# jfjell/Octree-Raymarcher

Hardware: AMD Instinct MI355X
Metric: Mrays/s (primary+shadow) at 1920x1080, depth-12 SVO (higher is better)
Workload: dtype f32; 1 GPU; c3_1080p_depth12_4x1x4_shadow; depth_per_chunk=12, chunksize=128, nodes=99473656, bricks=34206642, hbm_pool_bytes=11087035656, kernel=auto, launches_in_flight=2, frames_per_launch=16, frames_in_flight=32, gather=False, partition=single, ranks_seen=1, launcher=single process

## Files before the change

include/svo.h:

```cpp
#ifndef SVO_H
#define SVO_H

#include <stdint.h>
#include <stddef.h>

#ifdef __cplusplus
extern "C" {
#endif

#define SVO_ABI_VERSION 4

typedef enum svo_status {
    SVO_OK                 =  0,
    SVO_OK_LITERAL_ONLY    =  1,
    SVO_ERR_INVALID_ARG    = -1,
    SVO_ERR_NO_DEVICE      = -2,
    SVO_ERR_OUT_OF_MEMORY  = -3,
    SVO_ERR_MALFORMED_TREE = -4,
    SVO_ERR_NOT_UPLOADED   = -5,
    SVO_ERR_UNSUPPORTED    = -6,
    SVO_ERR_HIP            = -7
} svo_status;

enum { SVO_EMPTY = 0, SVO_LEAF = 1, SVO_BRANCH = 2, SVO_TWIG = 3 };
// ... 51 lines not shown
    int32_t  max_tree_steps;
    int32_t  max_twig_steps;
    int32_t  shadow;
    float    light_dir[3];
    int32_t  kernel;
    int32_t  tiles_per_wave;
    uint32_t *counters_dev;
    int32_t  normal_mode;
    int32_t  launches_in_flight;
    uint32_t       *tile_cost_dev;
    const uint32_t *tile_order_dev;
    int32_t  semantics;
    uint32_t see_through;
} svo_trace_params;
enum { SVO_NORMAL_CUBE = 0, SVO_NORMAL_FACE = 1 };
enum { SVO_SHADOW_NO_CLEARANCE = 2 };
enum { SVO_SEMANTICS_CPU = 0, SVO_SEMANTICS_GLSL = 1 };

enum {
    SVO_HIT_FLAG      = 1u << 0,
    SVO_SHADOW_TRACED = 1u << 1,
    SVO_SHADOWED      = 1u << 2,
    SVO_FACE_NORMAL   = 1u << 3,
    SVO_SEE_THROUGH   = 1u << 4,
    SVO_LOCAL_SHADOWS  = 1u << 5,
    SVO_SHADOWED_POINT = 1u << 6,
    SVO_SHADOWED_SPOT  = 1u << 7,
    SVO_ERR_FLAG      = 1u << 15
};
#define SVO_CELL_NONE 0xFFu

// ... 207 lines not shown
    float    alpha;
    uint32_t style;
    uint32_t _pad[3];
} svo_box;

int svo_cursor_place(const float origin[3], const float dir[3], const svo_hit *record_dev,
                     float size, svo_box *box_dev, void *stream);

int svo_shade_boxes(const svo_camera *cam, const svo_box *boxes_dev, int nboxes, float near_plane, float far_plane,
                    int x0, int y0, int w, int h, float *rgba_dev, void *stream);

int svo_trace_last_ray_count(svo_world *, void *stream, uint64_t *rays);

int svo_world_prepare_light(svo_world *, const float light_dir[3], void *stream);
int svo_world_prepared_light(svo_world *, void *stream, float shadow_dir[3], uint64_t *clear_nodes);

int   svo_device_count(void);
void *svo_device_alloc(size_t bytes);
void  svo_device_free(void *p_dev);
void  svo_device_cache_trim(void);
int   svo_memcpy_h2d(void *dst_dev, const void *src, size_t bytes);
int   svo_memcpy_d2h(void *dst, const void *src_dev, size_t bytes);
int   svo_stream_synchronize(void *stream);

const char *svo_last_error(void);
int         svo_abi_version(void);

#ifdef __cplusplus
}
#endif
// ... 2 lines not shown
```

octree-raymarcher_amd/__init__.py:

```python
from __future__ import annotations

import ctypes as C
import math
import os
from typing import Optional, Sequence

import numpy as np

from . import partition

_HERE = os.path.dirname(os.path.abspath(__file__))
LIB_PATH = os.environ.get("SVO_AMD_LIB") or os.path.join(_HERE, "libsvo_amd.so")

if not os.path.exists(LIB_PATH):
    raise ImportError(
        f"{LIB_PATH} is missing: build it with `make -C {_HERE}` (or __graft_entry__.build()). "
        "There is no CPU fallback for the SVO march.")

lib = C.CDLL(LIB_PATH)

SVO_OK = 0
OK_LITERAL_ONLY = 1
ERR_NAMES = {0: "SVO_OK", -1: "SVO_ERR_INVALID_ARG", -2: "SVO_ERR_NO_DEVICE", -3: "SVO_ERR_OUT_OF_MEMORY",
             -4: "SVO_ERR_MALFORMED_TREE", -5: "SVO_ERR_NOT_UPLOADED", -6: "SVO_ERR_UNSUPPORTED", -7: "SVO_ERR_HIP"}
EMPTY, LEAF, BRANCH, TWIG = 0, 1, 2, 3
KERNEL_AUTO, KERNEL_LITERAL, KERNEL_STACK = 0, 1, 2
EDIT_BUILD, EDIT_DESTROY, EDIT_REPLACE = 0, 1, 2
HIT_FLAG, SHADOW_TRACED, SHADOWED, FACE_NORMAL, SEE_THROUGH, ERR_FLAG = 1, 2, 4, 8, 16, 1 << 15
LOCAL_SHADOWS, SHADOWED_POINT, SHADOWED_SPOT = 1 << 5, 1 << 6, 1 << 7
NORMAL_CUBE, NORMAL_FACE = 0, 1
SHADOW_NO_CLEARANCE = 2
SEMANTICS_CPU, SEMANTICS_GLSL = 0, 1
CELL_NONE = 0xFF
SKY_LINEAR, SKY_NEAREST = 0, 1
BOX_SOLID, BOX_CURSOR, BOX_HIDDEN = 0, 1, 1 << 8
MAX_BOXES = 64
BOX_DTYPE = np.dtype([("bmin", "<f4", (3,)), ("size", "<f4"), ("color", "<f4", (3,)), ("alpha", "<f4"), ("style", "<u4"), ("_pad", "<u4", (3,))])
assert BOX_DTYPE.itemsize == 48

HIT_DTYPE = np.dtype([("t", "<f4"), ("normal", "<f4", (3,)), ("material", "<u2"), ("flags", "<u2"),
                      ("chunk", "<u4"), ("node", "<u4"), ("cell", "<u4")])
assert HIT_DTYPE.itemsize == 32
LOCATE_INSIDE, LOCATE_SOLID = 1, 2
VOXEL_DTYPE = np.dtype([("bmin", "<f4", (3,)), ("size", "<f4"), ("material", "<u2"), ("flags", "<u2"),
                        ("chunk", "<u4"), ("node", "<u4"), ("cell", "<u4")])
assert VOXEL_DTYPE.itemsize == 32
# ... 99 lines not shown
                ("total_trees", C.c_uint64), ("total_twigs", C.c_uint64),
                ("tree_pool_bytes", C.c_uint64), ("twig_pool_bytes", C.c_uint64), ("mask_pool_bytes", C.c_uint64),
                ("max_chunk_depth", C.c_int32), ("exact_geometry", C.c_int32),
                ("wide_pool_bytes", C.c_uint64), ("wide_nodes", C.c_uint64)]


MAX_FRAMES = 16

ABI_SYMBOLS = [
    "svo_world_generate", "svo_world_create", "svo_world_info_get", "svo_world_chunk", "svo_world_destroy",
    "svo_world_index_float", "svo_world_index", "svo_world_locate", "svo_hit_voxels", "svo_hit_uv", "svo_shade_textured", "svo_world_upload", "svo_world_update",
    "svo_chunk_from_grid", "svo_world_chunk_from_grid", "svo_world_chunk_to_grid",
    "svo_chunk_write", "svo_chunk_read", "svo_chunk_free", "svo_world_shift", "svo_world_edit_box", "svo_world_edit_cube", "svo_world_edit_ball", "svo_world_edit_ball_all", "svo_world_compact", "svo_world_coarsen", "svo_shade", "svo_shade_packed", "svo_shade_translucent", "svo_shade_sky", "svo_frame_rgba8", "svo_cursor_place", "svo_shade_boxes", "svo_shade_defaults", "svo_gbuffer_pack", "svo_gbuffer_unpack",
    "svo_tile_order", "svo_trace", "svo_trace_rows", "svo_trace_frames", "svo_trace_rows_frames", "svo_trace_rays", "svo_trace_segments", "svo_trace_translucent", "svo_trace_local_shadows", "svo_trace_last_ray_count",
    "svo_shadowmap_fit", "svo_shadowmap_render", "svo_shadowmap_apply", "svo_hit_ao", "svo_shade_ao",
    "svo_trace_reflections", "svo_shade_reflections", "svo_world_prepare_light", "svo_world_prepared_light",
    "svo_device_count", "svo_device_alloc", "svo_device_free", "svo_device_cache_trim", "svo_memcpy_h2d", "svo_memcpy_d2h",
    "svo_stream_synchronize", "svo_last_error", "svo_abi_version",
]

_P = C.c_void_p
lib.svo_last_error.restype = C.c_char_p
lib.svo_abi_version.restype = C.c_int
lib.svo_world_edit_box.argtypes = [_P, C.c_int, C.c_int, C.POINTER(C.c_float), C.POINTER(C.c_float), C.c_uint16]
lib.svo_world_edit_cube.argtypes = [_P, C.c_int, C.POINTER(C.c_float), C.c_float, C.c_uint16, C.POINTER(C.c_int), C.POINTER(C.c_int)]
lib.svo_world_edit_ball.argtypes = [_P, C.c_int, C.c_int, C.POINTER(C.c_float), C.c_float, C.c_uint16]
lib.svo_world_edit_ball_all.argtypes = [_P, C.c_int, C.POINTER(C.c_float), C.c_float, C.c_uint16, C.POINTER(C.c_int), C.c_int, C.POINTER(C.c_int)]
lib.svo_world_compact.argtypes = [_P, C.c_int]
lib.svo_world_compact.restype = C.c_int
lib.svo_world_coarsen.argtypes = [_P, C.c_int]
lib.svo_world_coarsen.restype = C.c_int
# ... 38 lines not shown
lib.svo_world_locate.argtypes = [_P, _P, C.c_int64, C.POINTER(TraceParams), _P, _P]
lib.svo_hit_voxels.argtypes = [_P, _P, C.c_int64, _P, _P]
lib.svo_hit_uv.argtypes = [C.POINTER(Camera), C.c_float, C.c_int, C.c_int, C.c_int, C.c_int, _P, _P, _P, _P]
lib.svo_shade_textured.argtypes = [C.POINTER(Camera), C.POINTER(ShadeParams), C.POINTER(Atlas), C.c_int, C.c_int, C.c_int, C.c_int, _P, _P, _P, _P]
lib.svo_hit_ao.argtypes = [_P, C.POINTER(Camera), C.POINTER(TraceParams), C.c_float, C.c_int, C.c_int, C.c_int, C.c_int, _P, _P, _P, _P]
lib.svo_shade_ao.argtypes = [_P, C.c_float, C.c_int64, _P, _P]
lib.svo_trace_reflections.argtypes = [_P, C.POINTER(Camera), C.POINTER(TraceParams), C.c_uint32, C.c_int, C.c_int, C.c_int, C.c_int, _P, _P, _P, _P]
lib.svo_shade_reflections.argtypes = [C.POINTER(Camera), C.POINTER(ShadeParams), C.POINTER(Mirror), C.c_int, C.c_int, C.c_int, C.c_int, _P, _P, _P, _P, _P]
lib.svo_shade_sky.argtypes = [C.POINTER(Camera), C.POINTER(Sky), C.c_int, C.c_int, C.c_int, C.c_int, _P, _P, _P, _P]
lib.svo_frame_rgba8.argtypes = [_P, C.c_int64, _P, _P]
lib.svo_cursor_place.argtypes = [C.POINTER(C.c_float), C.POINTER(C.c_float), _P, C.c_float, _P, _P]
lib.svo_shade_boxes.argtypes = [C.POINTER(Camera), _P, C.c_int, C.c_float, C.c_float, C.c_int, C.c_int, C.c_int, C.c_int, _P, _P]
lib.svo_trace_last_ray_count.argtypes = [_P, _P, C.POINTER(C.c_uint64)]
lib.svo_world_prepare_light.argtypes = [_P, C.POINTER(C.c_float), _P]
lib.svo_world_prepared_light.argtypes = [_P, _P, C.POINTER(C.c_float), C.POINTER(C.c_uint64)]
lib.svo_device_count.restype = C.c_int
lib.svo_device_alloc.argtypes = [C.c_size_t]
lib.svo_device_alloc.restype = _P
lib.svo_device_free.argtypes = [_P]
lib.svo_device_free.restype = None
lib.svo_device_cache_trim.argtypes = []
lib.svo_device_cache_trim.restype = None
lib.svo_memcpy_h2d.argtypes = [_P, _P, C.c_size_t]
lib.svo_memcpy_d2h.argtypes = [_P, _P, C.c_size_t]
lib.svo_stream_synchronize.argtypes = [_P]


def _check(rc: int, where: str) -> int:
    if rc < 0:
        raise SvoError(rc, where)
# ... 62 lines not shown
def default_camera(world_w: int, world_d: int, chunksize: int, width: int, height: int) -> Camera:
    cx = world_w * chunksize * 0.5
    return make_camera((cx, 150.0, -40.0), (0.0, -0.5, 0.866), (0.0, 1.0, 0.0), 60.0, width, height)


def c5_scene() -> dict:
    return {
        "generate": dict(pyramid_resolution=4096, water=False, coarse_depth=10, refine_box=((62.0, -1e9, -1e9), (66.0, 1e9, 1e9))),
        "camera": lambda w, h: make_camera((64.3, 12.7, 96.5), (0.0, -0.8, 0.6), (0.0, 1.0, 0.0), 60.0, w, h),
    }


def trace_params(shadow: bool = False, kernel: int = KERNEL_AUTO, light_dir=(1.0, -1.0, 0.0), eps: float = 0.0,
                 caps=(0, 0, 0), counters_dev: Optional[int] = None, tiles_per_wave: int = 0, normal_mode: int = 0,
                 tile_cost_dev: Optional[int] = None, tile_order_dev: Optional[int] = None, launches_in_flight: int = 0,
                 semantics: int = 0, see_through: int = 0, light_clearance: bool = True) -> TraceParams:
    p = TraceParams()
    p.semantics = semantics
    p.see_through = see_through
    p.normal_mode = normal_mode
    p.eps = eps
    p.max_chunk_steps, p.max_tree_steps, p.max_twig_steps = caps
    p.shadow = (1 if light_clearance else 1 | SHADOW_NO_CLEARANCE) if shadow else 0
    p.light_dir[:] = [float(x) for x in light_dir]
    p.kernel = kernel
    p.counters_dev = counters_dev
    p.tiles_per_wave = tiles_per_wave
    p.tile_cost_dev = tile_cost_dev
    p.tile_order_dev = tile_order_dev
    p.launches_in_flight = launches_in_flight
    return p


def chunk_write(path: str, chunk: dict, treestoragesize: int = 0, twigstoragesize: int = 0):
    tree = np.ascontiguousarray(chunk["tree"], dtype=np.uint32)
    twig = np.ascontiguousarray(chunk["twig"], dtype=np.uint16)
    d = ChunkDesc()
    d.position[:] = [float(x) for x in chunk["position"]]
# ... 337 lines not shown

    def shadowmap_render(self, smap: ShadowMap, params: TraceParams, stream: int = 0):
        _check(lib.svo_shadowmap_render(self._h, C.byref(smap) if smap is not None else None, C.byref(params) if params is not None else None,
                                        stream), "svo_shadowmap_render")

    def tile_order(self, cost_ptr: int, order_ptr: int, ntiles: int, stream: int = 0):
        _check(lib.svo_tile_order(self._h, cost_ptr, order_ptr, ntiles, stream), "svo_tile_order")

    def prepare_light(self, light_dir=(1.0, -1.0, 0.0), stream: int = 0):
        _check(lib.svo_world_prepare_light(self._h, (C.c_float * 3)(*[float(v) for v in light_dir]), stream), "svo_world_prepare_light")

    def prepared_light(self, stream: int = 0):
        sdir, n = (C.c_float * 3)(), C.c_uint64()
        _check(lib.svo_world_prepared_light(self._h, stream, sdir, C.byref(n)), "svo_world_prepared_light")
        return tuple(sdir), n.value

    def last_ray_count(self, stream: int = 0) -> int:
        n = C.c_uint64()
        _check(lib.svo_trace_last_ray_count(self._h, stream, C.byref(n)), "svo_trace_last_ray_count")
        return n.value

    def draw(self, cam: Camera, rect=None, shadow: bool = False, kernel: int = KERNEL_AUTO, counters: bool = False,
             light_dir=(1.0, -1.0, 0.0), normal_mode: int = 0, semantics: int = 0, see_through: int = 0, local_shadows=None, shadowmap=None):
        x0, y0, w, h = rect if rect is not None else (0, 0, cam.width, cam.height)
        out = DeviceBuffer(max(w * h, 1) * 32)
        cnt = DeviceBuffer(max(w * h, 1) * 16) if counters else None
        prm = trace_params(shadow=shadow, kernel=kernel, light_dir=light_dir, counters_dev=cnt.ptr if cnt else None, normal_mode=normal_mode,
                           semantics=semantics, see_through=see_through)
        if shadowmap is not None:
            prm.shadow = 0
# ... 120 lines not shown
```

octree-raymarcher_amd/csrc/device.hip:

```cpp
#include <hip/hip_runtime.h>

#include <algorithm>
#include <cmath>
#include <cstdlib>
#include <chrono>
#include <cstring>
#include <mutex>
#include <new>
#include <string>
#include <vector>

#include "kernel_literal.hip.h"
#include "kernel_stack.hip.h"
#include "see_through.hip.h"
#include "local_shadows.hip.h"
#include "reflect.hip.h"
#include "shadowmap.hip.h"
#include "locate.hip.h"
#include "ao.hip.h"
#include "hit_voxels.hip.h"
#include "hip_own.h"
#include "wide_tree.hip.h"
#include "light_clearance.hip.h"

// ... 12 lines not shown
#pragma unroll
    for (int k = 0; k < 4; ++k) {
        const uint32_t a = w[k] & 0xFFFFu, b = w[k] >> 16;
        bits |= (a ? 1u : 0u) << (2 * k);
        bits |= (b ? 1u : 0u) << (2 * k + 1);
        if (a) { lo = a < lo ? a : lo; hi = a > hi ? a : hi; }
        if (b) { lo = b < lo ? b : lo; hi = b > hi ? b : hi; }
    }
#pragma unroll
    for (int d = 1; d < 8; d <<= 1) {
        const uint32_t lo2 = __shfl_xor(lo, d, 64), hi2 = __shfl_xor(hi, d, 64);
        lo = lo2 < lo ? lo2 : lo; hi = hi2 > hi ? hi2 : hi;
    }
    if (!live) return;
    reinterpret_cast<uint8_t *>(mask + first)[i] = (uint8_t)bits;
    if ((i & 7u) == 0u) bmat[first + (i >> 3)] = (uint16_t)(hi == 0u ? 0u : (lo == hi ? lo : 0xFFFFu));
}

__global__ __launch_bounds__(256) void k_tile_keys(const uint32_t *cost, uint32_t *keys, uint32_t *idx, int n)
{
    const int i = blockIdx.x * 256 + threadIdx.x;
    if (i >= n) return;
    const uint32_t a = cost[2 * i], b = cost[2 * i + 1];
    keys[i] = a + b < a ? 0xFFFFFFFFu : a + b;
    idx[i] = (uint32_t)i;
}

constexpr size_t POOL_CACHE_SLOTS = 8, POOL_CACHE_MIN = 1u << 20;
struct PoolBuf { void *p; size_t bytes; int device; };
static std::mutex g_pool_mutex;
static std::vector<PoolBuf> g_pool_cache;
// ... 49 lines not shown
    w.hbm->view_wide = Pooled<uint32_t>(); w.hbm->view_mask = Pooled<uint64_t>(); w.hbm->view_material = 0;
}

static void drop_parents(svo_world &w)
{
    Hbm &d = *w.hbm;
    if (d.parent.p || d.parent_level.p || d.chunk_trees.p) (void)hipDeviceSynchronize();
    d.parent = Pooled<uint32_t>(); d.parent_level = Pooled<uint8_t>(); d.chunk_trees = DevBuf<uint32_t>();
    d.parents_ok = false;
}

static void drop_clearance(svo_world &w)
{
    Hbm &d = *w.hbm;
    if (d.clear_place.p) { (void)hipDeviceSynchronize(); d.clear_place = Pooled<uint4>(); }
    d.clear_state = Hbm::CLEAR_DROPPED; d.clear_usable = false;
}

int release_device(svo_world &w, bool keep_builder)
{
    if (w.hbm) {
        (void)hipSetDevice(w.device);
        drop_view(w);
        drop_parents(w);
        if (!keep_builder) free_builder_context(w);
        (void)hipDeviceSynchronize();
        delete w.hbm;
        w.hbm = nullptr;
    }
    w.device = -1;
    w.table.clear(); w.tree_slot.clear(); w.twig_slot.clear(); w.wtable.clear(); w.wide_slot.clear();
// ... 696 lines not shown
    float m = 1.0f;
    for (int a = 0; a < 3; ++a)
        for (int k = 0; k < 2; ++k) m = std::max(m, std::fabs((float)(w.chunkcoordmin[a] + k * dims[a]) * (float)w.chunksize));
    return std::nextafter(m, INFINITY) - m;
}
static bool eps_is_pow2(float eps)
{
    uint32_t b;
    std::memcpy(&b, &eps, sizeof b);
    return (b & 0x807FFFFFu) == 0u && b >= 0x00800000u && b < 0x7F800000u;
}

static int prepare_light(svo_world &w, const float sdir[3], hipStream_t s)
{
    Hbm &d = *w.hbm;
    d.clear_usable = false;
    if (!w.wide_ok || w.wide_pool_len == 0) return SVO_OK;
    HIP_TRY(hipSetDevice(w.device));
    bool premises = true;
    for (int a = 0; a < 3; ++a) premises &= std::isfinite(sdir[a]) && (sdir[a] == 0.0f || std::fabs((double)sdir[a]) >= CLEAR_S_MIN);
    std::memcpy(d.clear_sdir, sdir, sizeof d.clear_sdir);
    d.clear_state = Hbm::CLEAR_READY;
    if (!premises || !w.exact_geometry) return SVO_OK;
    d.clear_state = Hbm::CLEAR_DROPPED;
    const uint64_t nodes = w.wide_pool_len;
    if (d.clear_place.bytes < nodes * sizeof(uint4)) {
        if (d.clear_place.p) HIP_TRY(hipDeviceSynchronize());
        if (d.clear_place.alloc(nodes, w.device) != hipSuccess) { set_error("svo_world_prepare_light: hipMalloc failed"); return SVO_ERR_OUT_OF_MEMORY; }
    }
    if (const int rc = d.clear_count.reserve(1, false, nullptr)) return rc;
    for (Event &e : d.work_done) if (e.e) if (const int rc = e.wait(s)) return rc;
    if (d.clear_built.e) if (const int rc = d.clear_built.wait(s)) return rc;
    const double u = (double)clear_spacing(w);
    ClearArgs K;
    K.wchunks = d.wchunks.p; K.wide = d.wide.p; K.place = d.clear_place.p; K.pool_nodes = nodes;
    K.n_chunks = (int32_t)w.chunks.size(); K.chunksize = (double)w.chunksize;
    for (int a = 0; a < 3; ++a) K.s[a] = (double)sdir[a];
    K.d1 = 4.0 * u;
    K.d2 = (8.0 / CLEAR_S_MIN + 6.0 + 4.0 * (double)(w.width + w.height + w.depth + 2)) * u;
    K.clear_nodes = d.clear_count.p;
    HIP_TRY(hipMemsetAsync(d.clear_place.p, 0xFF, nodes * sizeof(uint4), s));
    HIP_TRY(hipMemsetAsync(d.clear_count.p, 0, sizeof(unsigned long long), s));
    int rc = launch_per_element("svo_world_prepare_light", K.n_chunks, s, k_clear_seed, K);
    const int nw_max = w.max_levels ? (w.max_levels + 1) / 2 : 1;
    for (int r = 0; rc == SVO_OK && r + 1 < nw_max; ++r) rc = launch_per_element("svo_world_prepare_light", (int64_t)nodes * 64, s, k_clear_boxes, K, (uint32_t)r);
    if (rc == SVO_OK) rc = launch_per_element("svo_world_prepare_light", (int64_t)nodes * 64, s, k_clear_sweep, K);
    if (rc != SVO_OK) return rc;
    if ((rc = d.clear_built.record(s)) != SVO_OK) return rc;
    d.clear_state = Hbm::CLEAR_READY;
    d.clear_usable = true;
    d.clear_eps = 2.0f * (float)u;
    return SVO_OK;
}

static int use_light_clearance(svo_world *w, const svo_trace_params *prm, TraceArgs &A, uint32_t see, hipStream_t s)
{
    A.light_clear = 0;
    if (!A.shadow || !A.from_camera || A.tmax || see || A.glsl || A.tile_cost || (prm && (prm->shadow & SVO_SHADOW_NO_CLEARANCE))) return SVO_OK;
    Hbm &d = *w->hbm;
    if (d.clear_state == Hbm::CLEAR_FRESH && (double)w->wide_pool_len * 64.0 * (double)w->chunks.size() <= CLEAR_AUTO_WORK)
        if (const int rc = prepare_light(*w, A.sdir, s)) return rc;
    if (d.clear_state != Hbm::CLEAR_READY || !d.clear_usable) return SVO_OK;
    if (std::memcmp(d.clear_sdir, A.sdir, sizeof d.clear_sdir) != 0 || !eps_is_pow2(A.eps) || A.eps < d.clear_eps) return SVO_OK;
    if (const int rc = d.clear_built.wait(s)) return rc;
    A.light_clear = 1;
    return SVO_OK;
}

static int launch(svo_world *w, const svo_trace_params *prm, TraceArgs &A, hipStream_t s)
{
    const int kernel = pick_kernel(w, prm, A);
    if (kernel < 0) return kernel;
    HIP_TRY(hipSetDevice(w->device));
    const uint32_t see = prm ? prm->see_through : 0u;
    if (see && kernel == SVO_KERNEL_STACK) {
        const int rc = use_view(w, see, A, s);
        if (rc != SVO_OK) return rc;
    }
    if (kernel == SVO_KERNEL_STACK) if (const int rc = use_light_clearance(w, prm, A, see, s)) return rc;
    Hbm &d = *w->hbm;
// ... 438 lines not shown
    const Hbm &d = *w->hbm;
    shadow_dir[0] = shadow_dir[1] = shadow_dir[2] = 0.0f;
    *clear_nodes = 0;
    if (d.clear_state != Hbm::CLEAR_READY) return SVO_OK;
    std::memcpy(shadow_dir, d.clear_sdir, sizeof d.clear_sdir);
    if (!d.clear_usable) return SVO_OK;
    HIP_TRY(hipSetDevice(w->device));
    HIP_TRY(hipStreamSynchronize((hipStream_t)stream));
    if (d.clear_built.e) HIP_TRY(hipEventSynchronize(d.clear_built.e));
    unsigned long long v = 0;
    HIP_TRY(hipMemcpy(&v, d.clear_count.p, sizeof v, hipMemcpyDeviceToHost));
    *clear_nodes = v;
    return SVO_OK;
}

}
```

octree-raymarcher_amd/csrc/hip_own.h:

```cpp
#pragma once
#include <hip/hip_runtime.h>

#include <algorithm>
#include <cstring>
#include <string>
#include <utility>
#include <vector>

#include "world.h"

namespace svo {

inline int hip_status(hipError_t e)
{
    return e == hipErrorOutOfMemory ? SVO_ERR_OUT_OF_MEMORY : (e == hipErrorNoDevice || e == hipErrorInvalidDevice) ? SVO_ERR_NO_DEVICE : SVO_ERR_HIP;
}
#define HIP_TRY(expr)                                                                              \
    do { if (hipError_t e_ = (expr); e_ != hipSuccess) { svo::set_error(std::string(#expr) + ": " + hipGetErrorString(e_)); return svo::hip_status(e_); } } while (0)

inline unsigned blocks_for(uint64_t n, unsigned per) { return (unsigned)((n + per - 1) / per); }

inline int launch_status(const char *who)
{
    const hipError_t e = hipGetLastError();
// ... 139 lines not shown
    Event work_done[WORK_SLOTS];
    OrderedScratch<unsigned char> sort;
    OrderedScratch<float> cont;
    OrderedScratch<float> mirror;
    OrderedScratch<float> local;
    OrderedScratch<float> shadowmap;
    Pooled<uint32_t> view_wide; Pooled<uint64_t> view_mask;
    uint32_t view_material = 0;
    Event view_built;
    Pooled<uint32_t> parent; Pooled<uint8_t> parent_level; DevBuf<uint32_t> chunk_trees;
    bool parents_ok = false;
    Event parents_built;
    enum { CLEAR_FRESH = 0, CLEAR_READY = 1, CLEAR_DROPPED = 2 };
    int clear_state = CLEAR_FRESH;
    bool clear_usable = false;
    float clear_sdir[3] = { 0.0f, 0.0f, 0.0f }; float clear_eps = 0.0f;
    Pooled<uint4> clear_place; DevBuf<unsigned long long> clear_count;
    Event clear_built;
    int stack_blocks[24] = {};
};

}
```

octree-raymarcher_amd/csrc/kernel_stack.hip.h:

```cpp
#pragma once
#include "march.hip.h"
#include "step_asm.hip.h"

namespace svo {

constexpr int CW_ESCAPE_PENDING = (int)0x80000000;
enum : int { M_DONE = 0, M_WORLD = 1, M_HIT = 2, M_TREE = 3, M_TWIG = 4 };

constexpr int VOTE_WORLD = 8;
constexpr int VOTE_HIT = 16;
constexpr int VOTE_BUSY = 24;
constexpr int CREEP_SERIOUS = 6;
constexpr int CREEP_LANES = 8;
#define SVO_LIKELY(x) __builtin_expect(!!(x), 1)
#define SVO_UNLIKELY(x) __builtin_expect(!!(x), 0)
constexpr int STEP_EXTRA = 4;
constexpr int STEP_LANES = 8;
constexpr int DRAIN_STEPS = 8;
#ifndef SVO_SURE_MISS_WHEN
#define SVO_SURE_MISS_WHEN __builtin_amdgcn_readfirstlane(more ? 0 : 1)
#endif

__device__ __forceinline__ float recip_pow2(float x) { return __uint_as_float(0x7F000000u - __float_as_uint(x)); }

// ... 582 lines not shown
                node = wb[child ? 0u : 1u + ci] + (child ? ci : gi);
            }
            const uint32_t hitc = (uint32_t)cnt;
            V3 vlo;
            float vsize;
            uint32_t material;
            if (hitc == SVO_CELL_NONE) {
                const int low = (1 << (levels - plev)) - 1;
                vlo = mk(Blo.x + (float)(pux & ~low) * res, Blo.y + (float)(puy & ~low) * res, Blo.z + (float)(puz & ~low) * res);
                vsize = res * (float)(low + 1);
                material = word & 0xFFFFu;
            } else {
                vlo = mk(Blo.x + (float)(hitc & 3u) * res, Blo.y + (float)((hitc >> 2) & 3u) * res, Blo.z + (float)(hitc >> 4) * res);
                vsize = res;
                const unsigned long long brick = (unsigned long long)twig_off + (word & WIDE_PAYLOAD);
                material = A.bmat[brick];
                if (material == 0xFFFFu) material = A.twig[brick * TWIG_WORDS + hitc];
            }
            const V3 point = alpha + beta * (tw - eps);
            const bool face = A.normal_mode == SVO_NORMAL_FACE;
            const V3 n = face ? face_normal(point, vlo, vlo + vsize, beta) : cube_normal_pow2(point, vlo, vsize, eps);
            const uint32_t flags = SVO_HIT_FLAG | (A.shadow ? SVO_SHADOW_TRACED : 0u) | (face ? (uint32_t)SVO_FACE_NORMAL : 0u);
            store_hit(A.out, outk, tw, n, material, flags, (uint32_t)ci, node, hitc);
            if (want_cost) note_tile_cost(outk, guard);
            mode = M_DONE;
            if (A.shadow) {
                alpha = point; beta = sdir; g = sg;
                outk |= (int)0x80000000;
                if constexpr (SEG) far = __uint_as_float(0x7F800000u);
                tw = 0.0f; cw = 0; guard = 0; creepn = 0;
                bool hit = true;
                if (!inside(alpha, wlo, whi)) tw = (GLSL ? enter_glsl(alpha, g, wlo, whi, hit) : enter(alpha, beta, wlo, whi, hit)) + eps;
                mode = hit ? M_WORLD : M_DONE;
                rays_marched++;
            }
        } }
    }

    unsigned total = rays_marched;
    for (int off = 32; off > 0; off >>= 1) total += __shfl_down(total, off, 64);
    if (lane == 0 && total) atomicAdd(&A.work[1], (unsigned long long)total);
#ifdef SVO_STACK_TIMING
    unsigned busiest = n_lane_busy;
    for (int off = 32; off > 0; off >>= 1) busiest = max(busiest, (unsigned)__shfl_xor((int)busiest, off, 64));
    unsigned busiest_twig = n_lane_busy == busiest ? n_lane_twig : 0u;
    for (int off = 32; off > 0; off >>= 1) busiest_twig = max(busiest_twig, (unsigned)__shfl_xor((int)busiest_twig, off, 64));
    if (lane == 0 && A.counters) {
        uint4 c; c.x = (uint32_t)t_begin; c.y = (uint32_t)__builtin_amdgcn_s_memrealtime(); c.z = n_iters; c.w = total;
// ... 17 lines not shown
```

octree-raymarcher_amd/csrc/light_clearance.hip.h:

```cpp
#pragma once
#include <hip/hip_runtime.h>

#include "wide_tree.hip.h"

namespace svo {

struct ClearArgs {
    const DevWide *wchunks;
    uint32_t *wide;
    uint4 *place;
    uint64_t pool_nodes;
    int32_t n_chunks;
    double chunksize;
    double s[3];
    double d1, d2;
    unsigned long long *clear_nodes;
};

constexpr uint32_t CLEAR_NO_PLACE = 0xFFFFFFFFu;
constexpr int CLEAR_MAX_WIDE_LEVELS = (WIDE_MAX_LEVELS + 1) / 2;

__global__ __launch_bounds__(256) void k_clear_seed(ClearArgs K)
{
    const int i = blockIdx.x * 256 + threadIdx.x;
    if (i >= K.n_chunks) return;
    const uint32_t top = K.wchunks[i].wide_off;
    if (top < K.pool_nodes) K.place[top] = make_uint4(0u, 0u, 0u, (uint32_t)i << 4);
}

__global__ __launch_bounds__(256) void k_clear_boxes(ClearArgs K, uint32_t r)
{
    const uint64_t i = (uint64_t)blockIdx.x * 256 + threadIdx.x;
// ... 40 lines not shown
            if (K.s[a] <= 0.0 && !(lo[a] < C.hi[a])) oct = false;
        }
        if (oct && clear_prism(K, C, lo, hi, K.d1)) return true;
        bool inner = true;
        for (int a = 0; a < 3; ++a) inner &= lo[a] >= inner_lo[a] && hi[a] <= inner_hi[a];
        if (inner) return false;
    }
    for (int a = 0; a < 3; ++a) {
        const double g = K.s[a] == 0.0 ? 0.0 : K.d2;
        if (K.s[a] >= 0.0 && !(hi[a] >= C.lo[a] - g)) return false;
        if (K.s[a] <= 0.0 && !(lo[a] <= C.hi[a] + g)) return false;
    }
    return clear_prism(K, C, lo, hi, K.d2);
}

__device__ bool clear_occupied(const ClearArgs &K, const ClearCell &C, int j, bool own)
{
    const DevWide ch = K.wchunks[j];
    const int levels = (int)ch.levels, nw = levels ? (levels + 1) >> 1 : 1;
    const double res = K.chunksize / (double)(1u << levels);
    const double base[3] = { (double)ch.bmin[0], (double)ch.bmin[1], (double)ch.bmin[2] };
    double inner_lo[3], inner_hi[3], lo[3], hi[3];
    for (int a = 0; a < 3; ++a) { inner_lo[a] = base[a] + K.d2; inner_hi[a] = base[a] + K.chunksize - K.d2; lo[a] = base[a]; hi[a] = base[a] + K.chunksize; }
    if (!clear_meets(K, C, own, inner_lo, inner_hi, lo, hi)) return false;
    uint32_t node[CLEAR_MAX_WIDE_LEVELS + 1], cur[CLEAR_MAX_WIDE_LEVELS + 1], bx[CLEAR_MAX_WIDE_LEVELS + 1], by[CLEAR_MAX_WIDE_LEVELS + 1], bz[CLEAR_MAX_WIDE_LEVELS + 1];
    int k = 0;
    node[0] = 0u; cur[0] = 0u; bx[0] = by[0] = bz[0] = 0u;
    while (k >= 0) {
        if (cur[k] >= 64u) { --k; continue; }
        const uint32_t s = cur[k]++;
        const int sh = 2 * (nw - 1 - k);
        const uint32_t c[3] = { bx[k] | ((s & 3u) << sh), by[k] | (((s >> 2) & 3u) << sh), bz[k] | ((s >> 4) << sh) };
        if (((c[0] | c[1] | c[2]) >> levels) != 0u) continue;
        const uint64_t wn = (uint64_t)ch.wide_off + node[k];
        if (wn >= K.pool_nodes) return true;
        const uint32_t word = K.wide[wn * 64u + s];
        const uint32_t type = node_type(word);
        if (type == EMPTY) continue;
        uint32_t span = 1u << sh;
        if (type != BRANCH) { const uint32_t lv = (word >> WIDE_LEVEL_SHIFT) & ((1u << WIDE_LEVEL_BITS) - 1u); span = lv <= (uint32_t)levels ? 1u << (levels - lv) : span; }
        const double edge = res * (double)span;
        for (int a = 0; a < 3; ++a) { lo[a] = base[a] + (double)(c[a] & ~(span - 1u)) * res; hi[a] = lo[a] + edge; }
        if (!clear_meets(K, C, own, inner_lo, inner_hi, lo, hi)) continue;
        if (type != BRANCH || k + 1 >= nw) return true;
        ++k;
        node[k] = word & WIDE_PAYLOAD_MASK; cur[k] = 0u; bx[k] = c[0]; by[k] = c[1]; bz[k] = c[2];
    }
    return false;
}

__global__ __launch_bounds__(256) void k_clear_sweep(ClearArgs K)
{
    const uint64_t i = (uint64_t)blockIdx.x * 256 + threadIdx.x;
    if (i >= K.pool_nodes * 64u) return;
    const uint4 b = K.place[i >> 6];
    if (b.w == CLEAR_NO_PLACE) return;
    const uint32_t word = K.wide[i];
    if (node_type(word) != EMPTY) return;
// ... 14 lines not shown
    for (int a = 0; a < 3; ++a) { C.lo[a] = (double)ch.bmin[a] + (double)(c[a] & ~(span - 1u)) * res; C.hi[a] = C.lo[a] + (double)span * res; }
    bool clear = !clear_occupied(K, C, own, true);
    for (int j = 0; clear && j < K.n_chunks; ++j)
        if (j != own) clear = !clear_occupied(K, C, j, false);
    const uint32_t out = clear ? (word | WIDE_CLEAR_BIT) : (word & ~WIDE_CLEAR_BIT);
    if (!child) K.wide[i] = out;
    else {
        uint32_t *node = K.wide + (i & ~(uint64_t)63u);
        for (uint32_t g = 0; g < 8u; ++g) node[slot | (g & 1u) | ((g & 2u) << 1) | ((g & 4u) << 2)] = out;
    }
    if (level == 0 && !child && slot != 0u) clear = false;
    const unsigned long long voted = __ballot(clear);
    if (clear && (int)(threadIdx.x & 63u) == __ffsll((long long)voted) - 1) atomicAdd(K.clear_nodes, (unsigned long long)__popcll(voted));
}

}
```

octree-raymarcher_amd/csrc/svo_format.h:

```cpp
#pragma once
#include <stdint.h>

namespace svo {

enum : uint32_t { EMPTY = 0, LEAF = 1, BRANCH = 2, TWIG = 3 };
constexpr uint32_t TWIG_LEVELS = 2, TWIG_SIZE = 4, TWIG_WORDS = 64;
constexpr uint32_t OFFSET_MASK = 0x3FFFFFFFu;

constexpr uint32_t node_make(uint32_t type, uint32_t offset) { return (type << 30) | (offset & OFFSET_MASK); }
constexpr uint32_t node_type(uint32_t w) { return w >> 30; }
constexpr uint32_t node_offset(uint32_t w) { return w & OFFSET_MASK; }

constexpr uint32_t FILL_ACTION_BITS = 3;
constexpr uint64_t FILL_KIDS_LIMIT = 1ull << 28;
constexpr uint32_t fill_pack(uint32_t action, uint32_t kids) { return action | (kids << FILL_ACTION_BITS); }
constexpr uint32_t fill_action(uint32_t w) { return w & ((1u << FILL_ACTION_BITS) - 1u); }
constexpr uint32_t fill_kids(uint32_t w) { return w >> FILL_ACTION_BITS; }
static_assert(fill_kids(fill_pack(5u, (uint32_t)FILL_KIDS_LIMIT - 1u)) == FILL_KIDS_LIMIT - 1u && fill_action(fill_pack(5u, (uint32_t)FILL_KIDS_LIMIT - 1u)) == 5u,
              "the largest child-block index the fill admits survives the packing");

struct DevChunk {
    float    bmin[3];
    uint32_t levels;
    uint64_t tree_off;
// ... 49 lines not shown
    int32_t  shadow;
    int32_t  normal_mode;
    int32_t  glsl;
    float    guard_eps, leaf_back;
    float    sdir[3];
    void     *out;
    uint32_t *counters;
    unsigned long long *work;
    int32_t  ntiles, tiles_per_row;
    int32_t  exact_geometry;
    uint32_t *tile_cost;
    const uint32_t *tile_order;
    const float *tmax;
    int32_t  light_clear;
};

}
```

octree-raymarcher_amd/host/svo_world.hpp:

```cpp
#pragma once
#include <cmath>
#include <cstring>
#include <stdexcept>
#include <string>
#include <vector>

#include "../../include/svo.h"

namespace svo {

struct Error : std::runtime_error {
    int code;
    Error(int c, const std::string &where) : std::runtime_error(where + ": " + svo_last_error()), code(c) {}
};
inline void check(int rc, const char *where) { if (rc < 0) throw Error(rc, where); }

struct vec3 { float x, y, z; };
struct ivec3 { int x, y, z; };

class GBuffer {
public:
    GBuffer() = default;
    GBuffer(int w, int h) { resize(w, h); }
    ~GBuffer() { svo_device_free(dev_); }
// ... 106 lines not shown
    void draw_frames(const std::vector<Camera> &cams, GBuffer &out, bool shadow = false, const float light_dir[3] = nullptr, void *stream = nullptr)
    {
        if (cams.empty()) return;
        const int w = cams[0].width, h = cams[0].height;
        if (out.width != w || out.height != h * (int)cams.size()) out.resize(w, h * (int)cams.size());
        svo_trace_params p;
        std::memset(&p, 0, sizeof p);
        p.semantics = semantics;
        p.shadow = shadow ? 1 : 0;
        if (light_dir) std::memcpy(p.light_dir, light_dir, sizeof p.light_dir);
        std::vector<svo_camera> plain(cams.begin(), cams.end());
        check(svo_trace_frames(world_, plain.data(), (int)plain.size(), &p, 0, 0, w, h, out.device(), stream), "World::draw_frames");
    }

    void prepare_light(const float light_dir[3] = nullptr, void *stream = nullptr) { check(svo_world_prepare_light(world_, light_dir, stream), "World::prepare_light"); }

    void local_shadows(const Camera &cam, GBuffer &gbuffer, const float point_position[3], const float spot_position[3],
                       bool shadow = false, const float light_dir[3] = nullptr, void *stream = nullptr)
    {
        svo_trace_params p;
        std::memset(&p, 0, sizeof p);
        p.semantics = semantics;
        p.shadow = shadow ? 1 : 0;
        if (light_dir) std::memcpy(p.light_dir, light_dir, sizeof p.light_dir);
        check(svo_trace_local_shadows(world_, &cam, &p, point_position, spot_position, 0, 0, cam.width, cam.height, gbuffer.device(), stream),
              "World::local_shadows");
    }

    void shadowmap_fit(const float direction[3], int width, int height, ShadowMap &map) const
    {
// ... 198 lines not shown
```

Baseline: 8403 Mrays/s.

## Precompute per-brick light clearance to skip shadow rays from clear bricks

Extends the light-clearance precompute with a per-brick pass that marks single-material bricks whose empty cells all have an unobstructed path toward the light, storing the flag in the high bit of the brick material word. In the stack kernel, a primary hit inside a flagged brick whose shadow start point falls in an empty cell ends the ray instead of marching a shadow ray. This cuts shadow-march work for surface voxels already known to be lit. In exchange, the light-prepare step gets an extra costly kernel, material decoding in the hit path changes, and correctness rests on the new clearance test being conservative.

```diff
diff --git a/include/svo.h b/include/svo.h
--- a/include/svo.h
+++ b/include/svo.h
@@ -89,7 +89,7 @@
     uint32_t see_through;
 } svo_trace_params;
 enum { SVO_NORMAL_CUBE = 0, SVO_NORMAL_FACE = 1 };
-enum { SVO_SHADOW_NO_CLEARANCE = 2 };
+enum { SVO_SHADOW_NO_CLEARANCE = 2, SVO_SHADOW_NO_BRICK_CLEARANCE = 4 };
 enum { SVO_SEMANTICS_CPU = 0, SVO_SEMANTICS_GLSL = 1 };
 
 enum {
@@ -327,6 +327,7 @@
 
 int svo_world_prepare_light(svo_world *, const float light_dir[3], void *stream);
 int svo_world_prepared_light(svo_world *, void *stream, float shadow_dir[3], uint64_t *clear_nodes);
+int svo_world_prepared_bricks(svo_world *, void *stream, uint64_t *flagged);
 
 int   svo_device_count(void);
 void *svo_device_alloc(size_t bytes);
diff --git a/octree-raymarcher_amd/__init__.py b/octree-raymarcher_amd/__init__.py
--- a/octree-raymarcher_amd/__init__.py
+++ b/octree-raymarcher_amd/__init__.py
@@ -30,6 +30,7 @@
 LOCAL_SHADOWS, SHADOWED_POINT, SHADOWED_SPOT = 1 << 5, 1 << 6, 1 << 7
 NORMAL_CUBE, NORMAL_FACE = 0, 1
 SHADOW_NO_CLEARANCE = 2
+SHADOW_NO_BRICK_CLEARANCE = 4
 SEMANTICS_CPU, SEMANTICS_GLSL = 0, 1
 CELL_NONE = 0xFF
 SKY_LINEAR, SKY_NEAREST = 0, 1
@@ -159,7 +160,7 @@
     "svo_chunk_write", "svo_chunk_read", "svo_chunk_free", "svo_world_shift", "svo_world_edit_box", "svo_world_edit_cube", "svo_world_edit_ball", "svo_world_edit_ball_all", "svo_world_compact", "svo_world_coarsen", "svo_shade", "svo_shade_packed", "svo_shade_translucent", "svo_shade_sky", "svo_frame_rgba8", "svo_cursor_place", "svo_shade_boxes", "svo_shade_defaults", "svo_gbuffer_pack", "svo_gbuffer_unpack",
     "svo_tile_order", "svo_trace", "svo_trace_rows", "svo_trace_frames", "svo_trace_rows_frames", "svo_trace_rays", "svo_trace_segments", "svo_trace_translucent", "svo_trace_local_shadows", "svo_trace_last_ray_count",
     "svo_shadowmap_fit", "svo_shadowmap_render", "svo_shadowmap_apply", "svo_hit_ao", "svo_shade_ao",
-    "svo_trace_reflections", "svo_shade_reflections", "svo_world_prepare_light", "svo_world_prepared_light",
+    "svo_trace_reflections", "svo_shade_reflections", "svo_world_prepare_light", "svo_world_prepared_light", "svo_world_prepared_bricks",
     "svo_device_count", "svo_device_alloc", "svo_device_free", "svo_device_cache_trim", "svo_memcpy_h2d", "svo_memcpy_d2h",
     "svo_stream_synchronize", "svo_last_error", "svo_abi_version",
 ]
@@ -228,6 +229,7 @@
 lib.svo_trace_last_ray_count.argtypes = [_P, _P, C.POINTER(C.c_uint64)]
 lib.svo_world_prepare_light.argtypes = [_P, C.POINTER(C.c_float), _P]
 lib.svo_world_prepared_light.argtypes = [_P, _P, C.POINTER(C.c_float), C.POINTER(C.c_uint64)]
+lib.svo_world_prepared_bricks.argtypes = [_P, _P, C.POINTER(C.c_uint64)]
 lib.svo_device_count.restype = C.c_int
 lib.svo_device_alloc.argtypes = [C.c_size_t]
 lib.svo_device_alloc.restype = _P
@@ -320,7 +322,7 @@
 def trace_params(shadow: bool = False, kernel: int = KERNEL_AUTO, light_dir=(1.0, -1.0, 0.0), eps: float = 0.0,
                  caps=(0, 0, 0), counters_dev: Optional[int] = None, tiles_per_wave: int = 0, normal_mode: int = 0,
                  tile_cost_dev: Optional[int] = None, tile_order_dev: Optional[int] = None, launches_in_flight: int = 0,
-                 semantics: int = 0, see_through: int = 0, light_clearance: bool = True) -> TraceParams:
+                 semantics: int = 0, see_through: int = 0, light_clearance: bool = True, brick_clearance: bool = True) -> TraceParams:
     p = TraceParams()
     p.semantics = semantics
     p.see_through = see_through
@@ -328,6 +330,8 @@
     p.eps = eps
     p.max_chunk_steps, p.max_tree_steps, p.max_twig_steps = caps
     p.shadow = (1 if light_clearance else 1 | SHADOW_NO_CLEARANCE) if shadow else 0
+    if shadow and not brick_clearance:
+        p.shadow |= SHADOW_NO_BRICK_CLEARANCE
     p.light_dir[:] = [float(x) for x in light_dir]
     p.kernel = kernel
     p.counters_dev = counters_dev
@@ -695,6 +699,11 @@
         sdir, n = (C.c_float * 3)(), C.c_uint64()
         _check(lib.svo_world_prepared_light(self._h, stream, sdir, C.byref(n)), "svo_world_prepared_light")
         return tuple(sdir), n.value
+
+    def prepared_bricks(self, stream: int = 0) -> int:
+        n = C.c_uint64()
+        _check(lib.svo_world_prepared_bricks(self._h, stream, C.byref(n)), "svo_world_prepared_bricks")
+        return n.value
 
     def last_ray_count(self, stream: int = 0) -> int:
         n = C.c_uint64()
diff --git a/octree-raymarcher_amd/csrc/device.hip b/octree-raymarcher_amd/csrc/device.hip
--- a/octree-raymarcher_amd/csrc/device.hip
+++ b/octree-raymarcher_amd/csrc/device.hip
@@ -50,7 +50,7 @@
     }
     if (!live) return;
     reinterpret_cast<uint8_t *>(mask + first)[i] = (uint8_t)bits;
-    if ((i & 7u) == 0u) bmat[first + (i >> 3)] = (uint16_t)(hi == 0u ? 0u : (lo == hi ? lo : 0xFFFFu));
+    if ((i & 7u) == 0u) bmat[first + (i >> 3)] = (uint16_t)(hi == 0u ? 0u : (lo == hi && lo < BMAT_CLEAR_BIT ? lo : BMAT_SEVERAL));
 }
 
 __global__ __launch_bounds__(256) void k_tile_keys(const uint32_t *cost, uint32_t *keys, uint32_t *idx, int n)
@@ -130,7 +130,7 @@
 {
     Hbm &d = *w.hbm;
     if (d.clear_place.p) { (void)hipDeviceSynchronize(); d.clear_place = Pooled<uint4>(); }
-    d.clear_state = Hbm::CLEAR_DROPPED; d.clear_usable = false;
+    d.clear_state = Hbm::CLEAR_DROPPED; d.clear_usable = d.clear_bricks_usable = false;
 }
 
 int release_device(svo_world &w, bool keep_builder)
@@ -857,7 +857,7 @@
 static int prepare_light(svo_world &w, const float sdir[3], hipStream_t s)
 {
     Hbm &d = *w.hbm;
-    d.clear_usable = false;
+    d.clear_usable = d.clear_bricks_usable = false;
     if (!w.wide_ok || w.wide_pool_len == 0) return SVO_OK;
     HIP_TRY(hipSetDevice(w.device));
     bool premises = true;
@@ -871,7 +871,7 @@
         if (d.clear_place.p) HIP_TRY(hipDeviceSynchronize());
         if (d.clear_place.alloc(nodes, w.device) != hipSuccess) { set_error("svo_world_prepare_light: hipMalloc failed"); return SVO_ERR_OUT_OF_MEMORY; }
     }
-    if (const int rc = d.clear_count.reserve(1, false, nullptr)) return rc;
+    if (const int rc = d.clear_count.reserve(2, false, nullptr)) return rc;
     for (Event &e : d.work_done) if (e.e) if (const int rc = e.wait(s)) return rc;
     if (d.clear_built.e) if (const int rc = d.clear_built.wait(s)) return rc;
     const double u = (double)clear_spacing(w);
@@ -882,16 +882,22 @@
     K.d1 = 4.0 * u;
     K.d2 = (8.0 / CLEAR_S_MIN + 6.0 + 4.0 * (double)(w.width + w.height + w.depth + 2)) * u;
     K.clear_nodes = d.clear_count.p;
+    bool bricks = true;
+    for (int a = 0; a < 3; ++a) bricks &= w.chunkcoordmin[a] >= 0;
+    for (const ChunkPools &c : w.chunks) bricks &= std::ldexp((double)w.chunksize, -(int)c.depth) >= u;
+    K.mask = d.mask.p; K.bmat = d.bmat.p; K.clear_bricks = d.clear_count.p + 1; K.brick_premises = bricks ? 1 : 0;
     HIP_TRY(hipMemsetAsync(d.clear_place.p, 0xFF, nodes * sizeof(uint4), s));
-    HIP_TRY(hipMemsetAsync(d.clear_count.p, 0, sizeof(unsigned long long), s));
+    HIP_TRY(hipMemsetAsync(d.clear_count.p, 0, 2 * sizeof(unsigned long long), s));
     int rc = launch_per_element("svo_world_prepare_light", K.n_chunks, s, k_clear_seed, K);
     const int nw_max = w.max_levels ? (w.max_levels + 1) / 2 : 1;
     for (int r = 0; rc == SVO_OK && r + 1 < nw_max; ++r) rc = launch_per_element("svo_world_prepare_light", (int64_t)nodes * 64, s, k_clear_boxes, K, (uint32_t)r);
     if (rc == SVO_OK) rc = launch_per_element("svo_world_prepare_light", (int64_t)nodes * 64, s, k_clear_sweep, K);
+    if (rc == SVO_OK) rc = launch_per_element("svo_world_prepare_light", (int64_t)nodes * 64, s, k_clear_bricks, K);
     if (rc != SVO_OK) return rc;
     if ((rc = d.clear_built.record(s)) != SVO_OK) return rc;
     d.clear_state = Hbm::CLEAR_READY;
     d.clear_usable = true;
+    d.clear_bricks_usable = bricks;
     d.clear_eps = 2.0f * (float)u;
     return SVO_OK;
 }
@@ -906,7 +912,8 @@
     if (d.clear_state != Hbm::CLEAR_READY || !d.clear_usable) return SVO_OK;
     if (std::memcmp(d.clear_sdir, A.sdir, sizeof d.clear_sdir) != 0 || !eps_is_pow2(A.eps) || A.eps < d.clear_eps) return SVO_OK;
     if (const int rc = d.clear_built.wait(s)) return rc;
-    A.light_clear = 1;
+    A.light_clear = LIGHT_CLEAR_NODES;
+    if (d.clear_bricks_usable && !(prm && (prm->shadow & SVO_SHADOW_NO_BRICK_CLEARANCE))) A.light_clear |= LIGHT_CLEAR_BRICKS;
     return SVO_OK;
 }
 
@@ -1375,4 +1382,20 @@
     return SVO_OK;
 }
 
-}
+int svo_world_prepared_bricks(svo_world *w, void *stream, uint64_t *flagged)
+{
+    if (!w || !flagged) return SVO_ERR_INVALID_ARG;
+    if (w->device < 0) { set_error("svo_world_prepared_bricks: world is not uploaded"); return SVO_ERR_NOT_UPLOADED; }
+    const Hbm &d = *w->hbm;
+    *flagged = 0;
+    if (d.clear_state != Hbm::CLEAR_READY || !d.clear_usable || !d.clear_bricks_usable) return SVO_OK;
+    HIP_TRY(hipSetDevice(w->device));
+    HIP_TRY(hipStreamSynchronize((hipStream_t)stream));
+    if (d.clear_built.e) HIP_TRY(hipEventSynchronize(d.clear_built.e));
+    unsigned long long v = 0;
+    HIP_TRY(hipMemcpy(&v, d.clear_count.p + 1, sizeof v, hipMemcpyDeviceToHost));
+    *flagged = v;
+    return SVO_OK;
+}
+
+}
diff --git a/octree-raymarcher_amd/csrc/hip_own.h b/octree-raymarcher_amd/csrc/hip_own.h
--- a/octree-raymarcher_amd/csrc/hip_own.h
+++ b/octree-raymarcher_amd/csrc/hip_own.h
@@ -177,6 +177,7 @@
     enum { CLEAR_FRESH = 0, CLEAR_READY = 1, CLEAR_DROPPED = 2 };
     int clear_state = CLEAR_FRESH;
     bool clear_usable = false;
+    bool clear_bricks_usable = false;
     float clear_sdir[3] = { 0.0f, 0.0f, 0.0f }; float clear_eps = 0.0f;
     Pooled<uint4> clear_place; DevBuf<unsigned long long> clear_count;
     Event clear_built;
diff --git a/octree-raymarcher_amd/csrc/kernel_stack.hip.h b/octree-raymarcher_amd/csrc/kernel_stack.hip.h
--- a/octree-raymarcher_amd/csrc/kernel_stack.hip.h
+++ b/octree-raymarcher_amd/csrc/kernel_stack.hip.h
@@ -620,8 +620,8 @@
                 vlo = mk(Blo.x + (float)(hitc & 3u) * res, Blo.y + (float)((hitc >> 2) & 3u) * res, Blo.z + (float)(hitc >> 4) * res);
                 vsize = res;
                 const unsigned long long brick = (unsigned long long)twig_off + (word & WIDE_PAYLOAD);
-                material = A.bmat[brick];
-                if (material == 0xFFFFu) material = A.twig[brick * TWIG_WORDS + hitc];
+                const uint32_t bw = A.bmat[brick];
+                material = bw == 0xFFFFu ? A.twig[brick * TWIG_WORDS + hitc] : (bw & 0x7FFFu) | ((bw & 0x8000u) << 1);
             }
             const V3 point = alpha + beta * (tw - eps);
             const bool face = A.normal_mode == SVO_NORMAL_FACE;
@@ -637,7 +637,15 @@
                 tw = 0.0f; cw = 0; guard = 0; creepn = 0;
                 bool hit = true;
                 if (!inside(alpha, wlo, whi)) tw = (GLSL ? enter_glsl(alpha, g, wlo, whi, hit) : enter(alpha, beta, wlo, whi, hit)) + eps;
-                mode = hit ? M_WORLD : M_DONE;
+                bool settled = !GLSL && !SEG && (A.light_clear & LIGHT_CLEAR_BRICKS) != 0 && (material >> 16) != 0u;
+                if (settled) {
+                    const float inv_res = recip_pow2(res);
+                    const float fx = (point.x - Blo.x) * inv_res, fy = (point.y - Blo.y) * inv_res, fz = (point.z - Blo.z) * inv_res;
+                    const uint32_t ux = (uint32_t)(int)fx, uy = (uint32_t)(int)fy, uz = (uint32_t)(int)fz;
+                    settled = (fx >= 0.0f) & (fy >= 0.0f) & (fz >= 0.0f) & ((ux | uy | uz) <= 3u);
+                    settled = settled && ((bmask >> ((uz * 16u + uy * 4u + ux) & 63u)) & 1ull) == 0ull;
+                }
+                mode = hit && !settled ? M_WORLD : M_DONE;
                 rays_marched++;
             }
         } }
diff --git a/octree-raymarcher_amd/csrc/light_clearance.hip.h b/octree-raymarcher_amd/csrc/light_clearance.hip.h
--- a/octree-raymarcher_amd/csrc/light_clearance.hip.h
+++ b/octree-raymarcher_amd/csrc/light_clearance.hip.h
@@ -15,7 +15,13 @@
     double s[3];
     double d1, d2;
     unsigned long long *clear_nodes;
+    const uint64_t *mask;
+    uint16_t *bmat;
+    unsigned long long *clear_bricks;
+    int32_t brick_premises;
 };
+
+constexpr uint32_t BMAT_CLEAR_BIT = 0x8000u, BMAT_SEVERAL = 0xFFFFu;
 
 constexpr uint32_t CLEAR_NO_PLACE = 0xFFFFFFFFu;
 constexpr int CLEAR_MAX_WIDE_LEVELS = (WIDE_MAX_LEVELS + 1) / 2;
@@ -86,6 +92,7 @@
     return clear_prism(K, C, lo, hi, K.d2);
 }
 
+template <bool CELLS = false>
 __device__ bool clear_occupied(const ClearArgs &K, const ClearCell &C, int j, bool own)
 {
     const DevWide ch = K.wchunks[j];
@@ -114,6 +121,23 @@
         const double edge = res * (double)span;
         for (int a = 0; a < 3; ++a) { lo[a] = base[a] + (double)(c[a] & ~(span - 1u)) * res; hi[a] = lo[a] + edge; }
         if (!clear_meets(K, C, own, inner_lo, inner_hi, lo, hi)) continue;
+        if constexpr (CELLS) {
+            if (type == TWIG) {
+                if (((c[0] | c[1] | c[2]) & (span - 1u)) != 0u) continue;
+                unsigned long long m = K.mask[ch.twig_off + (word & WIDE_PAYLOAD_MASK)];
+                const double leaf = edge * 0.25, blo[3] = { lo[0], lo[1], lo[2] };
+                bool met = false;
+                while (m != 0ull && !met) {
+                    const uint32_t w = (uint32_t)__ffsll((long long)m) - 1u;
+                    m &= m - 1ull;
+                    lo[0] = blo[0] + leaf * (double)(w & 3u); lo[1] = blo[1] + leaf * (double)((w >> 2) & 3u); lo[2] = blo[2] + leaf * (double)(w >> 4);
+                    for (int a = 0; a < 3; ++a) hi[a] = lo[a] + leaf;
+                    met = clear_meets(K, C, own, inner_lo, inner_hi, lo, hi);
+                }
+                if (met) return true;
+                continue;
+            }
+        }
         if (type != BRANCH || k + 1 >= nw) return true;
         ++k;
         node[k] = word & WIDE_PAYLOAD_MASK; cur[k] = 0u; bx[k] = c[0]; by[k] = c[1]; bz[k] = c[2];
@@ -158,4 +182,51 @@
     if (clear && (int)(threadIdx.x & 63u) == __ffsll((long long)voted) - 1) atomicAdd(K.clear_nodes, (unsigned long long)__popcll(voted));
 }
 
-}
+__global__ __launch_bounds__(256) void k_clear_bricks(ClearArgs K)
+{
+    const uint64_t wn = ((uint64_t)blockIdx.x * 256 + threadIdx.x) >> 6;
+    if (wn >= K.pool_nodes) return;
+    const uint4 b = K.place[wn];
+    if (b.w == CLEAR_NO_PLACE) return;
+    const uint32_t lane = threadIdx.x & 63u;
+    const int own = (int)(b.w >> 4), k = (int)(b.w & 15u);
+    const DevWide ch = K.wchunks[own];
+    const int levels = (int)ch.levels, nw = levels ? (levels + 1) >> 1 : 1;
+    const int sh = 2 * (nw - 1 - k);
+    const double res = K.chunksize / (double)(1u << levels);
+    unsigned long long twigs = __ballot(node_type(K.wide[wn * 64u + lane]) == TWIG);
+    unsigned flagged = 0;
+    while (twigs != 0ull) {
+        const uint32_t slot = (uint32_t)__ffsll((long long)twigs) - 1u;
+        twigs &= twigs - 1ull;
+        const uint32_t word = K.wide[wn * 64u + slot];
+        const uint32_t c[3] = { b.x | ((slot & 3u) << sh), b.y | (((slot >> 2) & 3u) << sh), b.z | ((slot >> 4) << sh) };
+        if (((c[0] | c[1] | c[2]) >> levels) != 0u) continue;
+        const int level = (int)((word >> WIDE_LEVEL_SHIFT) & ((1u << WIDE_LEVEL_BITS) - 1u));
+        if (level > levels) continue;
+        const uint32_t span = 1u << (levels - level);
+        if (((c[0] | c[1] | c[2]) & (span - 1u)) != 0u) continue;
+        const uint64_t brick = ch.twig_off + (word & WIDE_PAYLOAD_MASK);
+        bool clear = K.brick_premises != 0;
+        if (clear && ((K.mask[brick] >> lane) & 1ull) == 0ull) {
+            const double leaf = res * (double)span * 0.25;
+            ClearCell C;
+            const uint32_t w3[3] = { lane & 3u, (lane >> 2) & 3u, lane >> 4 };
+            for (int a = 0; a < 3; ++a) { C.lo[a] = (double)ch.bmin[a] + (double)c[a] * res + leaf * (double)w3[a]; C.hi[a] = C.lo[a] + leaf; }
+            clear = !clear_occupied<true>(K, C, own, true);
+            for (int j = 0; clear && j < K.n_chunks; ++j)
+                if (j != own) clear = !clear_occupied<true>(K, C, j, false);
+        }
+        const bool all_clear = __ballot(!clear) == 0ull;
+        if (lane == 0u) {
+            const uint32_t m = K.bmat[brick];
+            if (m != BMAT_SEVERAL) {
+                K.bmat[brick] = (uint16_t)((m & ~BMAT_CLEAR_BIT) | (all_clear ? BMAT_CLEAR_BIT : 0u));
+                flagged += all_clear;
+            }
+        }
+    }
+    if (flagged) atomicAdd(K.clear_bricks, (unsigned long long)flagged);
+}
+
+}
diff --git a/octree-raymarcher_amd/csrc/svo_format.h b/octree-raymarcher_amd/csrc/svo_format.h
--- a/octree-raymarcher_amd/csrc/svo_format.h
+++ b/octree-raymarcher_amd/csrc/svo_format.h
@@ -87,5 +87,6 @@
     const float *tmax;
     int32_t  light_clear;
 };
+enum : int32_t { LIGHT_CLEAR_NODES = 1, LIGHT_CLEAR_BRICKS = 2 };
 
 }
diff --git a/octree-raymarcher_amd/host/svo_world.hpp b/octree-raymarcher_amd/host/svo_world.hpp
--- a/octree-raymarcher_amd/host/svo_world.hpp
+++ b/octree-raymarcher_amd/host/svo_world.hpp
@@ -144,6 +144,7 @@
     }
 
     void prepare_light(const float light_dir[3] = nullptr, void *stream = nullptr) { check(svo_world_prepare_light(world_, light_dir, stream), "World::prepare_light"); }
+    uint64_t prepared_bricks(void *stream = nullptr) { uint64_t n = 0; check(svo_world_prepared_bricks(world_, stream, &n), "World::prepared_bricks"); return n; }
 
     void local_shadows(const Camera &cam, GBuffer &gbuffer, const float point_position[3], const float spot_position[3],
                        bool shadow = false, const float light_dir[3] = nullptr, void *stream = nullptr)
```

After: 8777 Mrays/s (median of 6 runs). 4.5% higher.
